# stattlab/azplugins

Measured on AMD Instinct MI355X. Metric: particle-steps/sec, PerturbedLennardJones pair force, higher is better.
Workload: dtype f64

## Files before the change

azplugins_amd/csrc/pair_tiled.hpp:

```cpp
#pragma once

#include <type_traits>

#include "pair_kernel.hpp"
#include "pair_plan.hpp"

#ifndef AZP_TILED_WAVES_PER_SIMD
#define AZP_TILED_WAVES_PER_SIMD 4
#endif

namespace azp
{
#ifdef AZP_TIMELINE
extern __device__ unsigned long long g_timeline[8 * 4 * 16384];
#endif

struct TileDyn
    {
    uint32_t n_shells;
    uint32_t stale;
    };

struct TiledKArgs
    {
    PairKArgs p;
    const uint32_t* tile_nstage;
    const uint64_t* tile_head;
    const uint32_t* stage_idx;
    const uint32_t* slice_Kend;
    uint32_t n_shells;
    const uint64_t* slice_head;
    const uint4* cnl;
    const uint8_t* perm;
    const TileDyn* dyn;
    const uint32_t* dflag;
    const unsigned long long* dbits;
    const float* disp;
    double shell_w;
    double shell_winv;
    double bound_extra;
    };

__device__ __forceinline__ float wave_max_nonneg(float v)
    {
#pragma unroll
    for (int off = 32; off > 0; off >>= 1)
        v = fmaxf(v, __shfl_xor(v, off, 64));
    return v;
    }

__device__ __forceinline__ uint32_t tile_shells_for(double b, double shell_winv)
    {
    if (!(b >= 0.0))
        return PLAN_SHELLS;
    if (b == 0.0)
        return 0u;
    if (!(shell_winv > 0.0))
        return PLAN_SHELLS;
    const double n = ceil(2.0 * b * (1.0 + 1e-9) * shell_winv);
    return n >= (double)PLAN_SHELLS ? PLAN_SHELLS : (uint32_t)n;
    }

#define AZP_TILE_STRIDE(CAP) ((CAP) + 1)

constexpr int TILE_BATCH = 4;

struct TileBatch
    {
    double x[TILE_BATCH], y[TILE_BATCH], z[TILE_BATCH];
    uint32_t off[TILE_BATCH];
    };

inline void fill_local_bound(TiledKArgs& k, const PairPlan& plan, const azp_pair_args& args)
    {
    const bool local = args.d_displacement && args.has_displacement_bound && args.displacement_bound >= 0.0;
    k.disp = local ? args.d_displacement : nullptr;
    k.dflag = (args.d_stale_flag && args.d_displacement_sq_bits) ? args.d_stale_flag : nullptr;
    k.dbits = k.dflag ? args.d_displacement_sq_bits : nullptr;
    if (k.dflag)
        k.disp = nullptr;
    k.shell_w = plan.shell_width;
    k.shell_winv = plan.shell_width > 0.0 ? 1.0 / plan.shell_width : 0.0;
    k.bound_extra = args.displacement_bound_extra > 0.0 ? args.displacement_bound_extra : 0.0;
    }

template<int CAP, int H> __device__ __forceinline__ void tile_gather(TileBatch& b, const uint4& u, const char* bx)
    {
    constexpr int NB = TILE_BATCH;
    const uint32_t w0 = H ? u.z : u.x, w1 = H ? u.w : u.y;
    b.off[0] = w0 & 0xffffu;
    b.off[1] = w0 >> 16;
    b.off[2] = w1 & 0xffffu;
    b.off[3] = w1 >> 16;
#pragma unroll
    for (int e = 0; e < NB; ++e)
        {
        b.x[e] = *reinterpret_cast<const double*>(bx + b.off[e]);
        b.y[e] = *reinterpret_cast<const double*>(bx + b.off[e] + AZP_TILE_STRIDE(CAP) * 8);
        b.z[e] = *reinterpret_cast<const double*>(bx + b.off[e] + AZP_TILE_STRIDE(CAP) * 16);
        }
    }

template<class E, int CAP, bool VIRIAL, bool SINGLE, bool XPLOR, bool WRAP>
__device__ __forceinline__ void tile_compute(const TileBatch& b, const TiledKArgs& a, const char* bt,
                                             const typename E::Coeff* __restrict__ s_coeff,
                                             const double* __restrict__ s_ronsq, const typename E::Coeff& c0, double ronsq0,
                                             double rcutsq_max, const double3& pi, int typei, double& fx, double& fy,
                                             double& fz, double& pe, double (&v)[6], uint32_t& n_core, uint32_t& n_in, double (&es)[2])
    {
    typedef typename E::Coeff Coeff;
    constexpr int NB = TILE_BATCH;
    constexpr bool SPLIT = SINGLE && !XPLOR && E::kSplitEnergy;
    double dx[NB], dy[NB], dz[NB], rsq[NB];
    bool any_in = false;
#pragma unroll
    for (int e = 0; e < NB; ++e)
        {
        dx[e] = pi.x - b.x[e]; dy[e] = pi.y - b.y[e]; dz[e] = pi.z - b.z[e];
        if (WRAP)
            min_image(a.p.box, dx[e], dy[e], dz[e]);
        rsq[e] = __builtin_fma(dz[e], dz[e], __builtin_fma(dy[e], dy[e], dx[e] * dx[e]));
        if (WRAP)
            rsq[e] = (b.off[e] == 0) ? 1.0e60 : rsq[e];
        any_in = any_in || (rsq[e] < rcutsq_max);
        }
    const bool none_in = !__any(any_in);
    if (SPLIT ? __builtin_expect(none_in, 0) : none_in)
        return;
    double fd[NB];
    if constexpr (SPLIT)
        {
        double x[NB];
        E::rcp4(rsq, x);
        bool any_core = false;
#pragma unroll
        for (int e = 0; e < NB; ++e)
            any_core = any_core || E::in_core(c0, rsq[e]);
        if (!__any(any_core))
            {
            const bool count_in = c0.tail_add != 0.0;
#pragma unroll
            for (int e = 0; e < NB; ++e)
                E::eval_split_tail(c0, rsq[e], x[e], fd[e], es[0], es[1], n_in, count_in);
            }
        else
            {
#pragma unroll
            for (int e = 0; e < NB; ++e)
                E::eval_split(c0, rsq[e], x[e], fd[e], pe, n_core, n_in);
            }
        }
#pragma unroll
    for (int e = 0; e < NB; ++e)
        {
        double force_divr, pair_eng = 0.0;
        if constexpr (SPLIT)
            force_divr = fd[e];
        else if (SINGLE)
            {
            const bool evaluated = E::eval(c0, rsq[e], force_divr, pair_eng);
            if (XPLOR && evaluated)
                apply_xplor(rsq[e], ronsq0, c0.rcutsq, force_divr, pair_eng);
            }
        else
            {
            const int typej = *reinterpret_cast<const int*>(bt + (b.off[e] >> 1));
            const uint32_t tp = (uint32_t)typei * a.p.ntypes + (uint32_t)typej;
            const Coeff cc = s_coeff[tp];
            const bool evaluated = E::eval(cc, rsq[e], force_divr, pair_eng);
            if (XPLOR && evaluated)
                apply_xplor(rsq[e], s_ronsq[tp], cc.rcutsq, force_divr, pair_eng);
            }
        fx = __builtin_fma(dx[e], force_divr, fx);
        fy = __builtin_fma(dy[e], force_divr, fy);
        fz = __builtin_fma(dz[e], force_divr, fz);
        if constexpr (!SPLIT)
            pe += pair_eng;
        if (VIRIAL)
            {
            const double fxx = force_divr * dx[e], fyy = force_divr * dy[e];
            v[0] = __builtin_fma(fxx, dx[e], v[0]);
            v[1] = __builtin_fma(fxx, dy[e], v[1]);
            v[2] = __builtin_fma(fxx, dz[e], v[2]);
            v[3] = __builtin_fma(fyy, dy[e], v[3]);
            v[4] = __builtin_fma(fyy, dz[e], v[4]);
            v[5] = __builtin_fma(force_divr * dz[e], dz[e], v[5]);
            }
        }
    }

template<class E, int TPP, int CAP, bool VIRIAL, bool SINGLE, bool XPLOR, bool WRAP>
__device__ __forceinline__ void tiled_loop(const TiledKArgs& a, const char* bx, const char* bt,
                                           const typename E::Coeff* __restrict__ s_coeff,
                                           const double* __restrict__ s_ronsq, const typename E::Coeff& c0, double ronsq0,
                                           double rcutsq_max, const char* __restrict__ slice_base, uint32_t lane_off, uint32_t Kb,
                                           double3 pi, int typei, double& fx, double& fy, double& fz, double& pe, double (&v)[6], uint32_t& n_core,
                                           uint32_t& n_in, double (&es)[2])
    {
    const uint4 zero4 = make_uint4(0, 0, 0, 0);
    auto chunk_at = [&](uint32_t kk) -> uint4
        { return *reinterpret_cast<const uint4*>(slice_base + (uint64_t)kk * 1024u + lane_off); };
    const uint32_t K = Kb >> 1;
    const uint32_t Kc = (Kb + 1u) >> 1;
    uint4 u = (Kc > 0) ? chunk_at(0) : zero4;
    uint4 un = (Kc > 1) ? chunk_at(1) : u;
    TileBatch A, B;
    tile_gather<CAP, 0>(A, u, bx);
    for (uint32_t kk = 0; kk < K; ++kk)
        {
        const uint4 un2 = chunk_at((kk + 2 < Kc) ? kk + 2 : Kc - 1);
        tile_gather<CAP, 1>(B, u, bx);
        __builtin_amdgcn_sched_barrier(0);
        tile_compute<E, CAP, VIRIAL, SINGLE, XPLOR, WRAP>(A, a, bt, s_coeff, s_ronsq, c0, ronsq0, rcutsq_max, pi, typei, fx, fy, fz, pe, v, n_core, n_in, es);
        __builtin_amdgcn_sched_barrier(0);
        tile_gather<CAP, 0>(A, un, bx);
        __builtin_amdgcn_sched_barrier(0);
        tile_compute<E, CAP, VIRIAL, SINGLE, XPLOR, WRAP>(B, a, bt, s_coeff, s_ronsq, c0, ronsq0, rcutsq_max, pi, typei, fx, fy, fz, pe, v, n_core, n_in, es);
        __builtin_amdgcn_sched_barrier(0);
        u = un;
        un = un2;
        }
    if (Kb & 1u)
        tile_compute<E, CAP, VIRIAL, SINGLE, XPLOR, WRAP>(A, a, bt, s_coeff, s_ronsq, c0, ronsq0, rcutsq_max, pi, typei, fx, fy, fz, pe, v, n_core, n_in, es);
    }

template<class E, int TPP, int CAP, bool VIRIAL, bool SINGLE, bool XPLOR>
__global__ void __launch_bounds__(256, E::kTileWaves) pair_forces_tiled_kernel(const TiledKArgs a, const typename E::Params* __restrict__ params)
    {
    typedef typename E::Coeff Coeff;
    constexpr int TB = 256 / TPP;
    constexpr int PW = 64 / TPP;
    extern __shared__ __attribute__((aligned(16))) unsigned char s_raw[];
    double* s_x = reinterpret_cast<double*>(s_raw);
    double* s_y = s_x + AZP_TILE_STRIDE(CAP);
    double* s_z = s_y + AZP_TILE_STRIDE(CAP);
    int* s_t = reinterpret_cast<int*>(s_z + AZP_TILE_STRIDE(CAP));
    Coeff* s_coeff = reinterpret_cast<Coeff*>(s_raw + (size_t)AZP_TILE_STRIDE(CAP) * 24 + (SINGLE ? 0 : (size_t)CAP * 4 + 8));
    double* s_ronsq = reinterpret_cast<double*>(s_coeff + (SINGLE ? 0 : a.p.ntypes * a.p.ntypes));

    const uint32_t tid = threadIdx.x;
    __builtin_amdgcn_s_setprio(3);
#ifdef AZP_TIMELINE
    const unsigned long long tl_t0 = __builtin_amdgcn_s_memrealtime();
    const unsigned long long tl_c0 = __builtin_amdgcn_s_memtime();
    unsigned long long tl_tb = 0, tl_tc = 0, tl_td = 0, tl_ta = 0;
#endif
    const uint32_t tile = a.p.first / TB + xcd_remap(blockIdx.x, a.p.nblocks_padded);
    const uint32_t first = tile * TB;
    if (first >= a.p.end)
        return;
    if (a.dyn && a.dyn->stale)
        return;
    if (a.dflag && *a.dflag)
        return;

    Coeff c0;
    double ronsq0 = 0.0;
    double rcutsq_max = 0.0;
    if (SINGLE)
        {
        c0 = to_uniform(prepare_coeff<E>(a.p, params, 0));
        if (XPLOR)
            ronsq0 = a.p.ronsq[0];
        rcutsq_max = c0.rcutsq;
        }
    else
        {
        const uint32_t ntp = a.p.ntypes * a.p.ntypes;
        for (uint32_t t = tid; t < ntp; t += 256)
            {
            s_coeff[t] = prepare_coeff<E>(a.p, params, t);
            s_ronsq[t] = XPLOR ? a.p.ronsq[t] : 0.0;
            }
        for (uint32_t t = 0; t < ntp; ++t)
            rcutsq_max = fmax(rcutsq_max, a.p.rcutsq[t]);
        }

#ifdef AZP_TIMELINE
    tl_ta = __builtin_amdgcn_s_memrealtime();
#endif
    const uint32_t n_stage = a.tile_nstage[tile];
    const uint32_t* __restrict__ stage = a.stage_idx + a.tile_head[tile];
    const double3 c = load_scalar3_of4(a.p.pos, first);
    if (tid == 0)
        {
        s_x[0] = PLAN_FAR; s_y[0] = PLAN_FAR; s_z[0] = PLAN_FAR;
        if (!SINGLE) s_t[0] = 0;
        }
    const uint32_t wave = (uint32_t)__builtin_amdgcn_readfirstlane((int)(tid >> 6)), lane = tid & 63;
    const uint32_t pl = lane / TPP;
    const uint32_t idx = first + ((TPP == 1 && a.perm) ? (uint32_t)a.perm[(uint64_t)tile * 256u + tid] : wave * PW + pl);
    const bool active = idx < a.p.end;
    const double4 own = load_scalar4(a.p.pos, active ? idx : first);
    const bool no_hint = !(a.p.r_list_max > 0.0);
    bool far_from_c = false;
    float dmax = a.disp ? a.disp[active ? idx : first] : 0.f;
    {
    constexpr int ROUNDS = (CAP + 255) / 256;
    uint32_t sj[ROUNDS];
#pragma unroll
    for (int r = 0; r < ROUNDS; ++r)
        {
        const uint32_t sidx = (uint32_t)r * 256u + tid;
        sj[r] = (sidx < n_stage) ? stage[sidx] : first;
        }
#ifdef AZP_TIMELINE
    __builtin_amdgcn_s_waitcnt(0);
    tl_tb = __builtin_amdgcn_s_memrealtime();
#endif
    double sxv[ROUNDS], syv[ROUNDS], szv[ROUNDS];
    int stv[ROUNDS];
    if (a.disp)
        {
#pragma unroll
        for (int r = 0; r < ROUNDS; ++r)
            dmax = fmaxf(dmax, a.disp[sj[r]]);
        }
#pragma unroll
    for (int r = 0; r < ROUNDS; ++r)
        {
        if (SINGLE)
            {
            const double3 pj = load_scalar3_of4(a.p.pos, sj[r]);
            sxv[r] = pj.x; syv[r] = pj.y; szv[r] = pj.z;
            }
        else
            {
            const double4 pj = load_scalar4(a.p.pos, sj[r]);
            sxv[r] = pj.x; syv[r] = pj.y; szv[r] = pj.z;
            stv[r] = type_from_w(pj.w);
            }
        }
#ifdef AZP_TIMELINE
    __builtin_amdgcn_s_waitcnt(0);
    tl_tc = __builtin_amdgcn_s_memrealtime();
#endif
#pragma unroll
    for (int r = 0; r < ROUNDS; ++r)
        {
        const uint32_t sidx = (uint32_t)r * 256u + tid;
        if (sidx < n_stage)
            {
            double x = sxv[r], y = syv[r], z = szv[r];
            if (!a.p.box.triclinic)
                {
                if (a.p.box.px) x = __builtin_fma(-a.p.box.Lx, rint((x - c.x) * a.p.box.Lxinv), x);
                if (a.p.box.py) y = __builtin_fma(-a.p.box.Ly, rint((y - c.y) * a.p.box.Lyinv), y);
                if (a.p.box.pz) z = __builtin_fma(-a.p.box.Lz, rint((z - c.z) * a.p.box.Lzinv), z);
                if (no_hint)
                    far_from_c = far_from_c || (a.p.box.px && fabs(x - c.x) >= 0.25 * a.p.box.Lx)
                                 || (a.p.box.py && fabs(y - c.y) >= 0.25 * a.p.box.Ly)
                                 || (a.p.box.pz && fabs(z - c.z) >= 0.25 * a.p.box.Lz);
                }
            s_x[sidx + 1] = x; s_y[sidx + 1] = y; s_z[sidx + 1] = z;
            if (!SINGLE)
                s_t[sidx + 1] = stv[r];
            }
        }
    }

    double3 pi = make_double3(0.0, 0.0, 0.0);
    int typei = 0;
    bool lane_wide = far_from_c || a.p.box.triclinic;
    if (active)
        {
        const double4 p = own;
        double x = p.x, y = p.y, z = p.z;
        if (!a.p.box.triclinic)
            {
            if (a.p.box.px) x = __builtin_fma(-a.p.box.Lx, rint((x - c.x) * a.p.box.Lxinv), x);
            if (a.p.box.py) y = __builtin_fma(-a.p.box.Ly, rint((y - c.y) * a.p.box.Lyinv), y);
            if (a.p.box.pz) z = __builtin_fma(-a.p.box.Lz, rint((z - c.z) * a.p.box.Lzinv), z);
            const double rx = no_hint ? 0.25 * a.p.box.Lx : a.p.r_list_max, ry = no_hint ? 0.25 * a.p.box.Ly : a.p.r_list_max,
                         rz = no_hint ? 0.25 * a.p.box.Lz : a.p.r_list_max;
            lane_wide = lane_wide || (a.p.box.px && fabs(x - c.x) + rx >= 0.5 * a.p.box.Lx)
                        || (a.p.box.py && fabs(y - c.y) + ry >= 0.5 * a.p.box.Ly)
                        || (a.p.box.pz && fabs(z - c.z) + rz >= 0.5 * a.p.box.Lz);
            }
        pi = make_double3(x, y, z);
        typei = type_from_w(p.w);
        }
#ifdef AZP_TIMELINE
    __builtin_amdgcn_s_waitcnt(0);
    tl_td = __builtin_amdgcn_s_memrealtime();
#endif
    __shared__ float s_dmax[4];
    if (a.disp)
        {
        dmax = wave_max_nonneg(dmax);
        if (lane == 0)
            s_dmax[wave] = dmax;
        }
    const bool wide = __syncthreads_or(lane_wide);
    __builtin_amdgcn_s_setprio(0);
#ifdef AZP_TIMELINE
    const unsigned long long tl_t1 = __builtin_amdgcn_s_memrealtime();
#endif
    uint32_t n_shells = a.dyn ? min(a.dyn->n_shells, PLAN_SHELLS) : a.n_shells;
    if (a.dbits)
        n_shells = tile_shells_for(to_uniform(sqrt(__longlong_as_double((long long)*a.dbits)) + a.bound_extra), a.shell_winv);
    if (a.disp)
        {
        const float d4 = fmaxf(fmaxf(s_dmax[0], s_dmax[1]), fmaxf(s_dmax[2], s_dmax[3]));
        n_shells = tile_shells_for(to_uniform((double)d4 + a.bound_extra), a.shell_winv);
        }

    const uint32_t slice = tile * 4 + wave;
    const uint32_t Kb = to_uniform(a.slice_Kend[(PLAN_SHELLS + 1) * slice + min(n_shells, PLAN_SHELLS)]);
    const uint64_t slice_head = to_uniform(a.slice_head[slice]);
    const char* __restrict__ slice_base = reinterpret_cast<const char*>(a.cnl + slice_head * 64ull);
    const uint32_t lane_off = lane * 16u;

    double fx = 0.0, fy = 0.0, fz = 0.0, pe = 0.0;
    double v[6] = {0.0, 0.0, 0.0, 0.0, 0.0, 0.0};
    uint32_t n_core = 0, n_in = 0;
    double es[2] = {0.0, 0.0};
    const char* bx = reinterpret_cast<const char*>(s_x);
    const char* bt = reinterpret_cast<const char*>(s_t);
    if (wide)
        tiled_loop<E, TPP, CAP, VIRIAL, SINGLE, XPLOR, true>(a, bx, bt, s_coeff, s_ronsq, c0, ronsq0, rcutsq_max, slice_base, lane_off, Kb, pi,
                                                            typei, fx, fy, fz, pe, v, n_core, n_in, es);
    else
        tiled_loop<E, TPP, CAP, VIRIAL, SINGLE, XPLOR, false>(a, bx, bt, s_coeff, s_ronsq, c0, ronsq0, rcutsq_max, slice_base, lane_off, Kb, pi,
                                                             typei, fx, fy, fz, pe, v, n_core, n_in, es);
    if constexpr (SINGLE && !XPLOR && E::kSplitEnergy)
        pe = E::finish_split(c0, pe, es[0], es[1], n_core, n_in);

#ifdef AZP_TIMELINE
    if (lane == 0 && tile < 16384)
        {
        unsigned long long* t = g_timeline + (tile * 4 + wave) * 8;
        t[4] = tl_ta; t[5] = tl_tb; t[6] = tl_tc; t[7] = tl_td;
        if (wave == 3)
            t[4] = __builtin_amdgcn_s_memtime() - tl_c0;
        t[0] = tl_t0; t[1] = tl_t1; t[2] = __builtin_amdgcn_s_memrealtime();
        t[3] = ((unsigned long long)__builtin_amdgcn_s_getreg((20 ) | (0 << 6) | (31 << 11)) << 32)
               | (unsigned)__builtin_amdgcn_s_getreg((4 ) | (0 << 6) | (31 << 11));
        }
#endif
    fx = group_sum<TPP>(fx);
    fy = group_sum<TPP>(fy);
    fz = group_sum<TPP>(fz);
    pe = group_sum<TPP>(pe);
    if (VIRIAL)
        {
#pragma unroll
        for (int cidx = 0; cidx < 6; ++cidx)
            v[cidx] = group_sum<TPP>(v[cidx]);
        }
    if (active && (lane % TPP) == 0)
        {
        store_scalar4(a.p.force, idx, fx, fy, fz, 0.5 * pe);
        if (VIRIAL)
            {
#pragma unroll
            for (int cidx = 0; cidx < 6; ++cidx)
                a.p.virial[(uint64_t)cidx * a.p.virial_pitch + idx] = 0.5 * v[cidx];
            }
        }
    }

inline TiledKArgs make_tiled_kargs(const PairPlan& plan, const azp_pair_args& args, const TileDyn* dyn, uint32_t tb)
    {
    TiledKArgs k = {};
    k.p = make_pair_kargs(args);
    k.tile_nstage = plan.d_tile_nstage;
    k.tile_head = plan.d_tile_head;
    k.stage_idx = plan.d_stage_idx;
    k.perm = plan.balanced ? plan.d_perm : nullptr;
    k.slice_Kend = plan.d_slice_Kend;
    k.n_shells = plan_shells_for(plan, args);
    fill_local_bound(k, plan, args);
    k.dyn = dyn;
    k.slice_head = plan.d_slice_head;
    k.cnl = plan.d_cnl;
    const uint32_t t0 = k.p.first / tb, t1 = (k.p.end + tb - 1) / tb;
    k.p.first = t0 * tb;
    k.p.end = (t1 * tb < args.N) ? t1 * tb : args.N;
    k.p.nblocks_padded = (t1 - t0 + 7u) & ~7u;
    return k;
    }

inline uint32_t plan_launch_cap(const PairPlan& plan, const azp_pair_args& args, uint32_t tb)
    {
    if (args.range_count == 0 || plan.h_tile_nstage.empty())
        return plan.cap;
    const uint32_t end = (args.range_first + args.range_count < args.N) ? args.range_first + args.range_count : args.N;
    const uint32_t t0 = args.range_first / tb, t1 = (end + tb - 1) / tb;
    uint32_t most = 0;
    for (uint32_t t = t0; t < t1 && t < plan.n_tiles; ++t)
        most = plan.h_tile_nstage[t] > most ? plan.h_tile_nstage[t] : most;
    return plan_cap_for(most);
    }

template<class E, int TPP, int CAP, bool VIRIAL, bool SINGLE>
int launch_tiled_instance(const PairPlan& plan, const azp_pair_args& args, const typename E::Params* d_params,
                          hipStream_t stream, const TileDyn* dyn)
    {
    const TiledKArgs k = make_tiled_kargs(plan, args, dyn, plan.tile);
    size_t lds = (size_t)AZP_TILE_STRIDE(CAP) * 24 + (SINGLE ? 0 : (size_t)CAP * 4 + 8);
    if (!SINGLE)
        lds += (sizeof(typename E::Coeff) + sizeof(double)) * (size_t)args.ntypes * args.ntypes;
    if (args.shift_mode == AZP_SHIFT_XPLOR)
        return launch_dyn_lds(pair_forces_tiled_kernel<E, TPP, CAP, VIRIAL, SINGLE, true>, k.p.nblocks_padded, 256, TPP, lds, stream, k, d_params);
    return launch_dyn_lds(pair_forces_tiled_kernel<E, TPP, CAP, VIRIAL, SINGLE, false>, k.p.nblocks_padded, 256, TPP, lds, stream, k, d_params);
    }

template<class E, int TPP, bool VIRIAL, bool SINGLE>
int launch_tiled_cap(const PairPlan& plan, const azp_pair_args& args, const typename E::Params* d_params, hipStream_t s, const TileDyn* dyn)
    {
    const uint32_t cap = plan_launch_cap(plan, args, plan.tile);
    switch (cap)
        {
    case 1024: return launch_tiled_instance<E, TPP, 1024, VIRIAL, SINGLE>(plan, args, d_params, s, dyn);
    case 1536: return launch_tiled_instance<E, TPP, 1536, VIRIAL, SINGLE>(plan, args, d_params, s, dyn);
    case 1664: return launch_tiled_instance<E, TPP, 1664, VIRIAL, SINGLE>(plan, args, d_params, s, dyn);
    case 2048: return launch_tiled_instance<E, TPP, 2048, VIRIAL, SINGLE>(plan, args, d_params, s, dyn);
    case 2560: return launch_tiled_instance<E, TPP, 2560, VIRIAL, SINGLE>(plan, args, d_params, s, dyn);
    default: return AZP_ERROR_INVALID_ARGUMENT;
        }
    }

template<class E>
int launch_tiled_tpp(const PairPlan& plan, const azp_pair_args& args, const typename E::Params* d_params, hipStream_t s, const TileDyn* dyn)
    {
    const bool single = (args.ntypes == 1);
    auto go = [&](auto t)
        {
        constexpr int TPP = decltype(t)::value;
        if (args.compute_virial)
            return single ? launch_tiled_cap<E, TPP, true, true>(plan, args, d_params, s, dyn)
                          : launch_tiled_cap<E, TPP, true, false>(plan, args, d_params, s, dyn);
        return single ? launch_tiled_cap<E, TPP, false, true>(plan, args, d_params, s, dyn)
                      : launch_tiled_cap<E, TPP, false, false>(plan, args, d_params, s, dyn);
        };
    switch (plan.tpp)
        {
    case 1: return go(std::integral_constant<int, 1>());
    case 2: return go(std::integral_constant<int, 2>());
    case 4: return go(std::integral_constant<int, 4>());
    default: return AZP_ERROR_INVALID_ARGUMENT;
        }
    }

}
```

Before: 9.013 billion.

## Add specialized single-type tiled path with core/tail phase split and fast staging

Adds a dedicated kernel path for TPP=1 single-type split-energy potentials that loads tile metadata through scalar (constant address space) loads, uses a fast periodic staging path with 32-bit offsets, and splits the neighbor chunk loop into a core phase and a tail phase. Chunks beyond a per-slice Kphase index are known to lie outside the WCA core given the displacement bound, so the tail phase skips the per-batch core test and wave vote. This cuts branch and vote overhead in the inner loop and setup latency, at the cost of more code, extra plan data (slice_Kphase) and a correctness dependence on the host-computed core reach bound.

```diff
diff --git a/azplugins_amd/csrc/pair_tiled.hpp b/azplugins_amd/csrc/pair_tiled.hpp
--- a/azplugins_amd/csrc/pair_tiled.hpp
+++ b/azplugins_amd/csrc/pair_tiled.hpp
@@ -39,6 +39,9 @@
     double shell_w;
     double shell_winv;
     double bound_extra;
+    const uint32_t* slice_Kphase;
+    double core_reach_sq;
+    uint32_t fast_stage;
     };
 
 __device__ __forceinline__ float wave_max_nonneg(float v)
@@ -59,6 +62,26 @@
         return PLAN_SHELLS;
     const double n = ceil(2.0 * b * (1.0 + 1e-9) * shell_winv);
     return n >= (double)PLAN_SHELLS ? PLAN_SHELLS : (uint32_t)n;
+    }
+
+template<class T> __device__ __forceinline__ T load_uniform(const T* p)
+    {
+    return *(const __attribute__((address_space(4))) T*)p;
+    }
+
+__device__ __forceinline__ double4 load_scalar4_o32(const double* base, uint32_t idx)
+    {
+    const char* p = reinterpret_cast<const char*>(base) + (idx << 5);
+    const double2 a = *reinterpret_cast<const double2*>(p);
+    const double2 b = *reinterpret_cast<const double2*>(p + 16);
+    return make_double4(a.x, a.y, b.x, b.y);
+    }
+__device__ __forceinline__ double3 load_scalar3_of4_o32(const double* base, uint32_t idx)
+    {
+    const char* p = reinterpret_cast<const char*>(base) + (idx << 5);
+    const double2 a = *reinterpret_cast<const double2*>(p);
+    const double z = *reinterpret_cast<const double*>(p + 16);
+    return make_double3(a.x, a.y, z);
     }
 
 #define AZP_TILE_STRIDE(CAP) ((CAP) + 1)
@@ -101,7 +124,7 @@
         }
     }
 
-template<class E, int CAP, bool VIRIAL, bool SINGLE, bool XPLOR, bool WRAP>
+template<class E, int CAP, bool VIRIAL, bool SINGLE, bool XPLOR, bool WRAP, bool TAIL = false>
 __device__ __forceinline__ void tile_compute(const TileBatch& b, const TiledKArgs& a, const char* bt,
                                              const typename E::Coeff* __restrict__ s_coeff,
                                              const double* __restrict__ s_ronsq, const typename E::Coeff& c0, double ronsq0,
@@ -133,15 +156,24 @@
         double x[NB];
         E::rcp4(rsq, x);
         bool any_core = false;
-#pragma unroll
-        for (int e = 0; e < NB; ++e)
-            any_core = any_core || E::in_core(c0, rsq[e]);
-        if (!__any(any_core))
+        if constexpr (!TAIL)
+            {
+#pragma unroll
+            for (int e = 0; e < NB; ++e)
+                any_core = any_core || E::in_core(c0, rsq[e]);
+            }
+        if (TAIL || !__any(any_core))
             {
             const bool count_in = c0.tail_add != 0.0;
 #pragma unroll
             for (int e = 0; e < NB; ++e)
-                E::eval_split_tail(c0, rsq[e], x[e], fd[e], es[0], es[1], n_in, count_in);
+                E::eval_split_tail(c0, rsq[e], x[e], fd[e], es[0], es[1], n_in, TAIL ? false : count_in);
+            if (TAIL && __builtin_expect(count_in, 0))
+                {
+#pragma unroll
+                for (int e = 0; e < NB; ++e)
+                    n_in += (rsq[e] < c0.rcutsq) ? 1u : 0u;
+                }
             }
         else
             {
@@ -224,240 +256,524 @@
         tile_compute<E, CAP, VIRIAL, SINGLE, XPLOR, WRAP>(A, a, bt, s_coeff, s_ronsq, c0, ronsq0, rcutsq_max, pi, typei, fx, fy, fz, pe, v, n_core, n_in, es);
     }
 
+template<class E, int TPP, int CAP, bool VIRIAL>
+__device__ __forceinline__ void tiled_loop_phases(const TiledKArgs& a, const char* bx, const typename E::Coeff& c0, double rcutsq_max,
+                                                  const char* __restrict__ slice_base, uint32_t lane_off, uint32_t Kb, uint32_t Kcore,
+                                                  double3 pi, int typei, double& fx, double& fy, double& fz, double& pe, double (&v)[6],
+                                                  uint32_t& n_core, uint32_t& n_in, double (&es)[2])
+    {
+    const uint4 zero4 = make_uint4(0, 0, 0, 0);
+    auto chunk_at = [&](uint32_t kk) -> uint4
+        { return *reinterpret_cast<const uint4*>(slice_base + (uint64_t)kk * 1024u + lane_off); };
+    const uint32_t K = Kb >> 1;
+    const uint32_t Kc = (Kb + 1u) >> 1;
+    uint4 u = (Kc > 0) ? chunk_at(0) : zero4;
+    uint4 un = (Kc > 1) ? chunk_at(1) : u;
+    TileBatch A, B;
+    tile_gather<CAP, 0>(A, u, bx);
+    auto iteration = [&](auto tail_tag, const uint32_t kk)
+        {
+        constexpr bool TAIL = decltype(tail_tag)::value;
+        const uint4 un2 = chunk_at((kk + 2 < Kc) ? kk + 2 : Kc - 1);
+        tile_gather<CAP, 1>(B, u, bx);
+        __builtin_amdgcn_sched_barrier(0);
+        tile_compute<E, CAP, VIRIAL, true, false, false, TAIL>(A, a, nullptr, nullptr, nullptr, c0, 0.0, rcutsq_max, pi, typei, fx, fy, fz, pe, v, n_core, n_in, es);
+        __builtin_amdgcn_sched_barrier(0);
+        tile_gather<CAP, 0>(A, un, bx);
+        __builtin_amdgcn_sched_barrier(0);
+        tile_compute<E, CAP, VIRIAL, true, false, false, TAIL>(B, a, nullptr, nullptr, nullptr, c0, 0.0, rcutsq_max, pi, typei, fx, fy, fz, pe, v, n_core, n_in, es);
+        __builtin_amdgcn_sched_barrier(0);
+        u = un;
+        un = un2;
+        };
+    const uint32_t K1 = (Kcore < K) ? Kcore : K;
+    for (uint32_t kk = 0; kk < K1; ++kk)
+        iteration(std::false_type(), kk);
+    for (uint32_t kk = K1; kk < K; ++kk)
+        iteration(std::true_type(), kk);
+    if (Kb & 1u)
+        tile_compute<E, CAP, VIRIAL, true, false, false>(A, a, nullptr, nullptr, nullptr, c0, 0.0, rcutsq_max, pi, typei, fx, fy, fz, pe, v, n_core, n_in, es);
+    }
 template<class E, int TPP, int CAP, bool VIRIAL, bool SINGLE, bool XPLOR>
 __global__ void __launch_bounds__(256, E::kTileWaves) pair_forces_tiled_kernel(const TiledKArgs a, const typename E::Params* __restrict__ params)
     {
-    typedef typename E::Coeff Coeff;
-    constexpr int TB = 256 / TPP;
-    constexpr int PW = 64 / TPP;
-    extern __shared__ __attribute__((aligned(16))) unsigned char s_raw[];
-    double* s_x = reinterpret_cast<double*>(s_raw);
-    double* s_y = s_x + AZP_TILE_STRIDE(CAP);
-    double* s_z = s_y + AZP_TILE_STRIDE(CAP);
-    int* s_t = reinterpret_cast<int*>(s_z + AZP_TILE_STRIDE(CAP));
-    Coeff* s_coeff = reinterpret_cast<Coeff*>(s_raw + (size_t)AZP_TILE_STRIDE(CAP) * 24 + (SINGLE ? 0 : (size_t)CAP * 4 + 8));
-    double* s_ronsq = reinterpret_cast<double*>(s_coeff + (SINGLE ? 0 : a.p.ntypes * a.p.ntypes));
-
-    const uint32_t tid = threadIdx.x;
-    __builtin_amdgcn_s_setprio(3);
-#ifdef AZP_TIMELINE
-    const unsigned long long tl_t0 = __builtin_amdgcn_s_memrealtime();
-    const unsigned long long tl_c0 = __builtin_amdgcn_s_memtime();
-    unsigned long long tl_tb = 0, tl_tc = 0, tl_td = 0, tl_ta = 0;
-#endif
-    const uint32_t tile = a.p.first / TB + xcd_remap(blockIdx.x, a.p.nblocks_padded);
-    const uint32_t first = tile * TB;
-    if (first >= a.p.end)
-        return;
-    if (a.dyn && a.dyn->stale)
-        return;
-    if (a.dflag && *a.dflag)
-        return;
-
-    Coeff c0;
-    double ronsq0 = 0.0;
-    double rcutsq_max = 0.0;
-    if (SINGLE)
-        {
-        c0 = to_uniform(prepare_coeff<E>(a.p, params, 0));
-        if (XPLOR)
-            ronsq0 = a.p.ronsq[0];
-        rcutsq_max = c0.rcutsq;
+    if constexpr (TPP == 1 && SINGLE && !XPLOR && E::kSplitEnergy)
+        {
+        typedef typename E::Coeff Coeff;
+        constexpr int TB = 256;
+        extern __shared__ __attribute__((aligned(16))) unsigned char s_raw[];
+        double* s_x = reinterpret_cast<double*>(s_raw);
+        double* s_y = s_x + AZP_TILE_STRIDE(CAP);
+        double* s_z = s_y + AZP_TILE_STRIDE(CAP);
+
+        const uint32_t tid = threadIdx.x;
+        __builtin_amdgcn_s_setprio(3);
+#ifdef AZP_TIMELINE
+        const unsigned long long tl_t0 = __builtin_amdgcn_s_memrealtime();
+        const unsigned long long tl_c0 = __builtin_amdgcn_s_memtime();
+        unsigned long long tl_tb = 0, tl_tc = 0, tl_td = 0, tl_ta = 0;
+#endif
+        const uint32_t tile = a.p.first / TB + xcd_remap(blockIdx.x, a.p.nblocks_padded);
+        const uint32_t first = tile * TB;
+        if (first >= a.p.end)
+            return;
+        const uint32_t wave = (uint32_t)__builtin_amdgcn_readfirstlane((int)(tid >> 6)), lane = tid & 63;
+        const uint32_t slice = tile * 4 + wave;
+
+        const uint32_t n_stage = load_uniform(a.tile_nstage + tile);
+        const uint64_t stage_head = load_uniform(a.tile_head + tile);
+        asm volatile("" ::"s"(n_stage), "s"(stage_head));
+        const uint32_t* __restrict__ stage = a.stage_idx + stage_head;
+        const uint32_t* spare = a.tile_nstage + tile;
+        const uint32_t w_stale = load_uniform(a.dyn ? &a.dyn->stale : spare);
+        const uint32_t w_shells = load_uniform(a.dyn ? &a.dyn->n_shells : spare);
+        const uint32_t w_flag = load_uniform(a.dflag ? a.dflag : spare);
+        const unsigned long long w_bits = load_uniform(a.dbits ? a.dbits : reinterpret_cast<const unsigned long long*>(a.tile_head + tile));
+        const double3 c = make_double3(load_uniform(a.p.pos + 4ull * first), load_uniform(a.p.pos + 4ull * first + 1),
+                                       load_uniform(a.p.pos + 4ull * first + 2));
+        const uint64_t slice_head = load_uniform(a.slice_head + slice);
+        const uint8_t member = *(a.perm ? a.perm + ((uint64_t)tile * 256u + tid) : reinterpret_cast<const uint8_t*>(spare));
+        constexpr int ROUNDS = (CAP + 255) / 256;
+        uint32_t sj[ROUNDS];
+#pragma unroll
+        for (int r = 0; r < ROUNDS; ++r)
+            {
+            const uint32_t sidx = (uint32_t)r * 256u + tid;
+            sj[r] = (sidx < n_stage) ? stage[sidx] : first;
+            }
+        __builtin_amdgcn_sched_barrier(0);
+        const uint32_t idx = first + (a.perm ? (uint32_t)member : wave * 64u + lane);
+        const bool active = idx < a.p.end;
+        if (((a.dyn != nullptr) & (w_stale != 0u)) | ((a.dflag != nullptr) & (w_flag != 0u)))
+            return;
+#ifdef AZP_TIMELINE
+        __builtin_amdgcn_s_waitcnt(0);
+        tl_tb = __builtin_amdgcn_s_memrealtime();
+#endif
+        uint32_t n_shells = a.dyn ? min(w_shells, PLAN_SHELLS) : a.n_shells;
+        if (a.dbits)
+            n_shells = tile_shells_for(to_uniform(sqrt(__longlong_as_double((long long)w_bits)) + a.bound_extra), a.shell_winv);
+        uint32_t Kb = load_uniform(a.slice_Kend + ((PLAN_SHELLS + 1) * slice + min(n_shells, PLAN_SHELLS)));
+        uint32_t Kcore = load_uniform(a.core_reach_sq > 0.0 ? a.slice_Kphase + slice : spare);
+
+        const Coeff c0 = to_uniform(E::prepare(params[0], load_uniform(a.p.rcutsq), a.p.shift_mode == AZP_SHIFT_SHIFT));
+        const double rcutsq_max = c0.rcutsq;
+        if (!(a.core_reach_sq > 0.0 && c0.wca_rsq <= a.core_reach_sq))
+            Kcore = 0xffffffffu;
+        asm volatile("" ::"s"(c.x), "s"(c.y), "s"(c.z), "s"(slice_head), "s"(Kb), "s"(Kcore), "s"(a.fast_stage), "s"(a.p.pos));
+        __builtin_amdgcn_sched_barrier(0);
+#ifdef AZP_TIMELINE
+        tl_ta = __builtin_amdgcn_s_memrealtime();
+#endif
+        if (tid == 0)
+            {
+            s_x[0] = PLAN_FAR; s_y[0] = PLAN_FAR; s_z[0] = PLAN_FAR;
+            }
+
+        double3 pi = make_double3(0.0, 0.0, 0.0);
+        bool lane_wide = false;
+        float dmax = 0.f;
+        const uint32_t me = active ? idx : first;
+        if (a.disp)
+            {
+            dmax = a.disp[me];
+#pragma unroll
+            for (int r = 0; r < ROUNDS; ++r)
+                dmax = fmaxf(dmax, a.disp[sj[r]]);
+            }
+        double sxv[ROUNDS], syv[ROUNDS], szv[ROUNDS];
+        if (a.fast_stage)
+            {
+            const double3 own = load_scalar3_of4_o32(a.p.pos, me);
+#pragma unroll
+            for (int r = 0; r < ROUNDS; ++r)
+                {
+                const double3 pj = load_scalar3_of4_o32(a.p.pos, sj[r]);
+                sxv[r] = pj.x; syv[r] = pj.y; szv[r] = pj.z;
+                }
+#ifdef AZP_TIMELINE
+            __builtin_amdgcn_s_waitcnt(0);
+            tl_tc = __builtin_amdgcn_s_memrealtime();
+#endif
+#pragma unroll
+            for (int r = 0; r < ROUNDS; ++r)
+                {
+                const uint32_t sidx = (uint32_t)r * 256u + tid;
+                if (sidx < n_stage)
+                    {
+                    s_x[sidx + 1] = __builtin_fma(-a.p.box.Lx, rint((sxv[r] - c.x) * a.p.box.Lxinv), sxv[r]);
+                    s_y[sidx + 1] = __builtin_fma(-a.p.box.Ly, rint((syv[r] - c.y) * a.p.box.Lyinv), syv[r]);
+                    s_z[sidx + 1] = __builtin_fma(-a.p.box.Lz, rint((szv[r] - c.z) * a.p.box.Lzinv), szv[r]);
+                    }
+                }
+            if (active)
+                {
+                const double x = __builtin_fma(-a.p.box.Lx, rint((own.x - c.x) * a.p.box.Lxinv), own.x);
+                const double y = __builtin_fma(-a.p.box.Ly, rint((own.y - c.y) * a.p.box.Lyinv), own.y);
+                const double z = __builtin_fma(-a.p.box.Lz, rint((own.z - c.z) * a.p.box.Lzinv), own.z);
+                lane_wide = (fabs(x - c.x) + a.p.r_list_max >= 0.5 * a.p.box.Lx) || (fabs(y - c.y) + a.p.r_list_max >= 0.5 * a.p.box.Ly)
+                            || (fabs(z - c.z) + a.p.r_list_max >= 0.5 * a.p.box.Lz);
+                pi = make_double3(x, y, z);
+                }
+            }
+        else
+            {
+            const double3 own = load_scalar3_of4(a.p.pos, me);
+            const bool no_hint = !(a.p.r_list_max > 0.0);
+            bool far_from_c = false;
+#pragma unroll
+            for (int r = 0; r < ROUNDS; ++r)
+                {
+                const double3 pj = load_scalar3_of4(a.p.pos, sj[r]);
+                sxv[r] = pj.x; syv[r] = pj.y; szv[r] = pj.z;
+                }
+#ifdef AZP_TIMELINE
+            __builtin_amdgcn_s_waitcnt(0);
+            tl_tc = __builtin_amdgcn_s_memrealtime();
+#endif
+#pragma unroll
+            for (int r = 0; r < ROUNDS; ++r)
+                {
+                const uint32_t sidx = (uint32_t)r * 256u + tid;
+                if (sidx < n_stage)
+                    {
+                    double x = sxv[r], y = syv[r], z = szv[r];
+                    if (!a.p.box.triclinic)
+                        {
+                        if (a.p.box.px) x = __builtin_fma(-a.p.box.Lx, rint((x - c.x) * a.p.box.Lxinv), x);
+                        if (a.p.box.py) y = __builtin_fma(-a.p.box.Ly, rint((y - c.y) * a.p.box.Lyinv), y);
+                        if (a.p.box.pz) z = __builtin_fma(-a.p.box.Lz, rint((z - c.z) * a.p.box.Lzinv), z);
+                        if (no_hint)
+                            far_from_c = far_from_c || (a.p.box.px && fabs(x - c.x) >= 0.25 * a.p.box.Lx)
+                                         || (a.p.box.py && fabs(y - c.y) >= 0.25 * a.p.box.Ly)
+                                         || (a.p.box.pz && fabs(z - c.z) >= 0.25 * a.p.box.Lz);
+                        }
+                    s_x[sidx + 1] = x; s_y[sidx + 1] = y; s_z[sidx + 1] = z;
+                    }
+                }
+            lane_wide = far_from_c || a.p.box.triclinic;
+            if (active)
+                {
+                double x = own.x, y = own.y, z = own.z;
+                if (!a.p.box.triclinic)
+                    {
+                    if (a.p.box.px) x = __builtin_fma(-a.p.box.Lx, rint((x - c.x) * a.p.box.Lxinv), x);
+                    if (a.p.box.py) y = __builtin_fma(-a.p.box.Ly, rint((y - c.y) * a.p.box.Lyinv), y);
+                    if (a.p.box.pz) z = __builtin_fma(-a.p.box.Lz, rint((z - c.z) * a.p.box.Lzinv), z);
+                    const double rx = no_hint ? 0.25 * a.p.box.Lx : a.p.r_list_max, ry = no_hint ? 0.25 * a.p.box.Ly : a.p.r_list_max,
+                                 rz = no_hint ? 0.25 * a.p.box.Lz : a.p.r_list_max;
+                    lane_wide = lane_wide || (a.p.box.px && fabs(x - c.x) + rx >= 0.5 * a.p.box.Lx)
+                                || (a.p.box.py && fabs(y - c.y) + ry >= 0.5 * a.p.box.Ly)
+                                || (a.p.box.pz && fabs(z - c.z) + rz >= 0.5 * a.p.box.Lz);
+                    }
+                pi = make_double3(x, y, z);
+                }
+            }
+#ifdef AZP_TIMELINE
+        __builtin_amdgcn_s_waitcnt(0);
+        tl_td = __builtin_amdgcn_s_memrealtime();
+#endif
+        __shared__ float s_dmax[4];
+        if (a.disp)
+            {
+            dmax = wave_max_nonneg(dmax);
+            if (lane == 0)
+                s_dmax[wave] = dmax;
+            }
+        const bool wide = __syncthreads_or(lane_wide);
+        __builtin_amdgcn_s_setprio(0);
+#ifdef AZP_TIMELINE
+        const unsigned long long tl_t1 = __builtin_amdgcn_s_memrealtime();
+#endif
+        if (a.disp)
+            {
+            const float d4 = fmaxf(fmaxf(s_dmax[0], s_dmax[1]), fmaxf(s_dmax[2], s_dmax[3]));
+            const uint32_t tile_shells = tile_shells_for(to_uniform((double)d4 + a.bound_extra), a.shell_winv);
+            Kb = to_uniform(a.slice_Kend[(PLAN_SHELLS + 1) * slice + min(tile_shells, PLAN_SHELLS)]);
+            }
+        const char* __restrict__ slice_base = reinterpret_cast<const char*>(a.cnl + slice_head * 64ull);
+        const uint32_t lane_off = lane * 16u;
+
+        double fx = 0.0, fy = 0.0, fz = 0.0, pe = 0.0;
+        double v[6] = {0.0, 0.0, 0.0, 0.0, 0.0, 0.0};
+        uint32_t n_core = 0, n_in = 0;
+        double es[2] = {0.0, 0.0};
+        const char* bx = reinterpret_cast<const char*>(s_x);
+        if (wide)
+            tiled_loop<E, 1, CAP, VIRIAL, true, false, true>(a, bx, nullptr, nullptr, nullptr, c0, 0.0, rcutsq_max, slice_base, lane_off, Kb, pi, 0,
+                                                             fx, fy, fz, pe, v, n_core, n_in, es);
+        else
+            tiled_loop_phases<E, 1, CAP, VIRIAL>(a, bx, c0, rcutsq_max, slice_base, lane_off, Kb, Kcore, pi, 0, fx, fy, fz, pe, v, n_core,
+                                                 n_in, es);
+        pe = E::finish_split(c0, pe, es[0], es[1], n_core, n_in);
+
+#ifdef AZP_TIMELINE
+        if (lane == 0 && tile < 16384)
+            {
+            unsigned long long* t = g_timeline + (tile * 4 + wave) * 8;
+            t[4] = tl_ta; t[5] = tl_tb; t[6] = tl_tc; t[7] = tl_td;
+            if (wave == 3)
+                t[4] = __builtin_amdgcn_s_memtime() - tl_c0;
+            t[0] = tl_t0; t[1] = tl_t1; t[2] = __builtin_amdgcn_s_memrealtime();
+            t[3] = ((unsigned long long)__builtin_amdgcn_s_getreg((20 ) | (0 << 6) | (31 << 11)) << 32)
+                   | (unsigned)__builtin_amdgcn_s_getreg((4 ) | (0 << 6) | (31 << 11));
+            }
+#endif
+        if (active)
+            {
+            store_scalar4(a.p.force, idx, fx, fy, fz, 0.5 * pe);
+            if (VIRIAL)
+                {
+#pragma unroll
+                for (int cidx = 0; cidx < 6; ++cidx)
+                    a.p.virial[(uint64_t)cidx * a.p.virial_pitch + idx] = 0.5 * v[cidx];
+                }
+            }
         }
     else
         {
-        const uint32_t ntp = a.p.ntypes * a.p.ntypes;
-        for (uint32_t t = tid; t < ntp; t += 256)
-            {
-            s_coeff[t] = prepare_coeff<E>(a.p, params, t);
-            s_ronsq[t] = XPLOR ? a.p.ronsq[t] : 0.0;
-            }
-        for (uint32_t t = 0; t < ntp; ++t)
-            rcutsq_max = fmax(rcutsq_max, a.p.rcutsq[t]);
-        }
-
-#ifdef AZP_TIMELINE
-    tl_ta = __builtin_amdgcn_s_memrealtime();
-#endif
-    const uint32_t n_stage = a.tile_nstage[tile];
-    const uint32_t* __restrict__ stage = a.stage_idx + a.tile_head[tile];
-    const double3 c = load_scalar3_of4(a.p.pos, first);
-    if (tid == 0)
-        {
-        s_x[0] = PLAN_FAR; s_y[0] = PLAN_FAR; s_z[0] = PLAN_FAR;
-        if (!SINGLE) s_t[0] = 0;
-        }
-    const uint32_t wave = (uint32_t)__builtin_amdgcn_readfirstlane((int)(tid >> 6)), lane = tid & 63;
-    const uint32_t pl = lane / TPP;
-    const uint32_t idx = first + ((TPP == 1 && a.perm) ? (uint32_t)a.perm[(uint64_t)tile * 256u + tid] : wave * PW + pl);
-    const bool active = idx < a.p.end;
-    const double4 own = load_scalar4(a.p.pos, active ? idx : first);
-    const bool no_hint = !(a.p.r_list_max > 0.0);
-    bool far_from_c = false;
-    float dmax = a.disp ? a.disp[active ? idx : first] : 0.f;
-    {
-    constexpr int ROUNDS = (CAP + 255) / 256;
-    uint32_t sj[ROUNDS];
-#pragma unroll
-    for (int r = 0; r < ROUNDS; ++r)
-        {
-        const uint32_t sidx = (uint32_t)r * 256u + tid;
-        sj[r] = (sidx < n_stage) ? stage[sidx] : first;
-        }
-#ifdef AZP_TIMELINE
-    __builtin_amdgcn_s_waitcnt(0);
-    tl_tb = __builtin_amdgcn_s_memrealtime();
-#endif
-    double sxv[ROUNDS], syv[ROUNDS], szv[ROUNDS];
-    int stv[ROUNDS];
-    if (a.disp)
-        {
+        typedef typename E::Coeff Coeff;
+        constexpr int TB = 256 / TPP;
+        constexpr int PW = 64 / TPP;
+        extern __shared__ __attribute__((aligned(16))) unsigned char s_raw[];
+        double* s_x = reinterpret_cast<double*>(s_raw);
+        double* s_y = s_x + AZP_TILE_STRIDE(CAP);
+        double* s_z = s_y + AZP_TILE_STRIDE(CAP);
+        int* s_t = reinterpret_cast<int*>(s_z + AZP_TILE_STRIDE(CAP));
+        Coeff* s_coeff = reinterpret_cast<Coeff*>(s_raw + (size_t)AZP_TILE_STRIDE(CAP) * 24 + (SINGLE ? 0 : (size_t)CAP * 4 + 8));
+        double* s_ronsq = reinterpret_cast<double*>(s_coeff + (SINGLE ? 0 : a.p.ntypes * a.p.ntypes));
+
+        const uint32_t tid = threadIdx.x;
+        __builtin_amdgcn_s_setprio(3);
+#ifdef AZP_TIMELINE
+        const unsigned long long tl_t0 = __builtin_amdgcn_s_memrealtime();
+        const unsigned long long tl_c0 = __builtin_amdgcn_s_memtime();
+        unsigned long long tl_tb = 0, tl_tc = 0, tl_td = 0, tl_ta = 0;
+#endif
+        const uint32_t tile = a.p.first / TB + xcd_remap(blockIdx.x, a.p.nblocks_padded);
+        const uint32_t first = tile * TB;
+        if (first >= a.p.end)
+            return;
+        if (a.dyn && a.dyn->stale)
+            return;
+        if (a.dflag && *a.dflag)
+            return;
+
+        Coeff c0;
+        double ronsq0 = 0.0;
+        double rcutsq_max = 0.0;
+        if (SINGLE)
+            {
+            c0 = to_uniform(prepare_coeff<E>(a.p, params, 0));
+            if (XPLOR)
+                ronsq0 = a.p.ronsq[0];
+            rcutsq_max = c0.rcutsq;
+            }
+        else
+            {
+            const uint32_t ntp = a.p.ntypes * a.p.ntypes;
+            for (uint32_t t = tid; t < ntp; t += 256)
+                {
+                s_coeff[t] = prepare_coeff<E>(a.p, params, t);
+                s_ronsq[t] = XPLOR ? a.p.ronsq[t] : 0.0;
+                }
+            for (uint32_t t = 0; t < ntp; ++t)
+                rcutsq_max = fmax(rcutsq_max, a.p.rcutsq[t]);
+            }
+
+#ifdef AZP_TIMELINE
+        tl_ta = __builtin_amdgcn_s_memrealtime();
+#endif
+        const uint32_t n_stage = a.tile_nstage[tile];
+        const uint32_t* __restrict__ stage = a.stage_idx + a.tile_head[tile];
+        const double3 c = load_scalar3_of4(a.p.pos, first);
+        if (tid == 0)
+            {
+            s_x[0] = PLAN_FAR; s_y[0] = PLAN_FAR; s_z[0] = PLAN_FAR;
+            if (!SINGLE) s_t[0] = 0;
+            }
+        const uint32_t wave = (uint32_t)__builtin_amdgcn_readfirstlane((int)(tid >> 6)), lane = tid & 63;
+        const uint32_t pl = lane / TPP;
+        const uint32_t idx = first + ((TPP == 1 && a.perm) ? (uint32_t)a.perm[(uint64_t)tile * 256u + tid] : wave * PW + pl);
+        const bool active = idx < a.p.end;
+        const double4 own = load_scalar4(a.p.pos, active ? idx : first);
+        const bool no_hint = !(a.p.r_list_max > 0.0);
+        bool far_from_c = false;
+        float dmax = a.disp ? a.disp[active ? idx : first] : 0.f;
+        {
+        constexpr int ROUNDS = (CAP + 255) / 256;
+        uint32_t sj[ROUNDS];
 #pragma unroll
         for (int r = 0; r < ROUNDS; ++r)
-            dmax = fmaxf(dmax, a.disp[sj[r]]);
-        }
-#pragma unroll
-    for (int r = 0; r < ROUNDS; ++r)
-        {
-        if (SINGLE)
-            {
-            const double3 pj = load_scalar3_of4(a.p.pos, sj[r]);
-            sxv[r] = pj.x; syv[r] = pj.y; szv[r] = pj.z;
-            }
-        else
-            {
-            const double4 pj = load_scalar4(a.p.pos, sj[r]);
-            sxv[r] = pj.x; syv[r] = pj.y; szv[r] = pj.z;
-            stv[r] = type_from_w(pj.w);
-            }
-        }
-#ifdef AZP_TIMELINE
-    __builtin_amdgcn_s_waitcnt(0);
-    tl_tc = __builtin_amdgcn_s_memrealtime();
-#endif
-#pragma unroll
-    for (int r = 0; r < ROUNDS; ++r)
-        {
-        const uint32_t sidx = (uint32_t)r * 256u + tid;
-        if (sidx < n_stage)
-            {
-            double x = sxv[r], y = syv[r], z = szv[r];
+            {
+            const uint32_t sidx = (uint32_t)r * 256u + tid;
+            sj[r] = (sidx < n_stage) ? stage[sidx] : first;
+            }
+#ifdef AZP_TIMELINE
+        __builtin_amdgcn_s_waitcnt(0);
+        tl_tb = __builtin_amdgcn_s_memrealtime();
+#endif
+        double sxv[ROUNDS], syv[ROUNDS], szv[ROUNDS];
+        int stv[ROUNDS];
+        if (a.disp)
+            {
+#pragma unroll
+            for (int r = 0; r < ROUNDS; ++r)
+                dmax = fmaxf(dmax, a.disp[sj[r]]);
+            }
+#pragma unroll
+        for (int r = 0; r < ROUNDS; ++r)
+            {
+            if (SINGLE)
+                {
+                const double3 pj = load_scalar3_of4(a.p.pos, sj[r]);
+                sxv[r] = pj.x; syv[r] = pj.y; szv[r] = pj.z;
+                }
+            else
+                {
+                const double4 pj = load_scalar4(a.p.pos, sj[r]);
+                sxv[r] = pj.x; syv[r] = pj.y; szv[r] = pj.z;
+                stv[r] = type_from_w(pj.w);
+                }
+            }
+#ifdef AZP_TIMELINE
+        __builtin_amdgcn_s_waitcnt(0);
+        tl_tc = __builtin_amdgcn_s_memrealtime();
+#endif
+#pragma unroll
+        for (int r = 0; r < ROUNDS; ++r)
+            {
+            const uint32_t sidx = (uint32_t)r * 256u + tid;
+            if (sidx < n_stage)
+                {
+                double x = sxv[r], y = syv[r], z = szv[r];
+                if (!a.p.box.triclinic)
+                    {
+                    if (a.p.box.px) x = __builtin_fma(-a.p.box.Lx, rint((x - c.x) * a.p.box.Lxinv), x);
+                    if (a.p.box.py) y = __builtin_fma(-a.p.box.Ly, rint((y - c.y) * a.p.box.Lyinv), y);
+                    if (a.p.box.pz) z = __builtin_fma(-a.p.box.Lz, rint((z - c.z) * a.p.box.Lzinv), z);
+                    if (no_hint)
+                        far_from_c = far_from_c || (a.p.box.px && fabs(x - c.x) >= 0.25 * a.p.box.Lx)
+                                     || (a.p.box.py && fabs(y - c.y) >= 0.25 * a.p.box.Ly)
+                                     || (a.p.box.pz && fabs(z - c.z) >= 0.25 * a.p.box.Lz);
+                    }
+                s_x[sidx + 1] = x; s_y[sidx + 1] = y; s_z[sidx + 1] = z;
+                if (!SINGLE)
+                    s_t[sidx + 1] = stv[r];
+                }
+            }
+        }
+
+        double3 pi = make_double3(0.0, 0.0, 0.0);
+        int typei = 0;
+        bool lane_wide = far_from_c || a.p.box.triclinic;
+        if (active)
+            {
+            const double4 p = own;
+            double x = p.x, y = p.y, z = p.z;
             if (!a.p.box.triclinic)
                 {
                 if (a.p.box.px) x = __builtin_fma(-a.p.box.Lx, rint((x - c.x) * a.p.box.Lxinv), x);
                 if (a.p.box.py) y = __builtin_fma(-a.p.box.Ly, rint((y - c.y) * a.p.box.Lyinv), y);
                 if (a.p.box.pz) z = __builtin_fma(-a.p.box.Lz, rint((z - c.z) * a.p.box.Lzinv), z);
-                if (no_hint)
-                    far_from_c = far_from_c || (a.p.box.px && fabs(x - c.x) >= 0.25 * a.p.box.Lx)
-                                 || (a.p.box.py && fabs(y - c.y) >= 0.25 * a.p.box.Ly)
-                                 || (a.p.box.pz && fabs(z - c.z) >= 0.25 * a.p.box.Lz);
-                }
-            s_x[sidx + 1] = x; s_y[sidx + 1] = y; s_z[sidx + 1] = z;
-            if (!SINGLE)
-                s_t[sidx + 1] = stv[r];
-            }
-        }
-    }
-
-    double3 pi = make_double3(0.0, 0.0, 0.0);
-    int typei = 0;
-    bool lane_wide = far_from_c || a.p.box.triclinic;
-    if (active)
-        {
-        const double4 p = own;
-        double x = p.x, y = p.y, z = p.z;
-        if (!a.p.box.triclinic)
-            {
-            if (a.p.box.px) x = __builtin_fma(-a.p.box.Lx, rint((x - c.x) * a.p.box.Lxinv), x);
-            if (a.p.box.py) y = __builtin_fma(-a.p.box.Ly, rint((y - c.y) * a.p.box.Lyinv), y);
-            if (a.p.box.pz) z = __builtin_fma(-a.p.box.Lz, rint((z - c.z) * a.p.box.Lzinv), z);
-            const double rx = no_hint ? 0.25 * a.p.box.Lx : a.p.r_list_max, ry = no_hint ? 0.25 * a.p.box.Ly : a.p.r_list_max,
-                         rz = no_hint ? 0.25 * a.p.box.Lz : a.p.r_list_max;
-            lane_wide = lane_wide || (a.p.box.px && fabs(x - c.x) + rx >= 0.5 * a.p.box.Lx)
-                        || (a.p.box.py && fabs(y - c.y) + ry >= 0.5 * a.p.box.Ly)
-                        || (a.p.box.pz && fabs(z - c.z) + rz >= 0.5 * a.p.box.Lz);
-            }
-        pi = make_double3(x, y, z);
-        typei = type_from_w(p.w);
-        }
-#ifdef AZP_TIMELINE
-    __builtin_amdgcn_s_waitcnt(0);
-    tl_td = __builtin_amdgcn_s_memrealtime();
-#endif
-    __shared__ float s_dmax[4];
-    if (a.disp)
-        {
-        dmax = wave_max_nonneg(dmax);
-        if (lane == 0)
-            s_dmax[wave] = dmax;
-        }
-    const bool wide = __syncthreads_or(lane_wide);
-    __builtin_amdgcn_s_setprio(0);
-#ifdef AZP_TIMELINE
-    const unsigned long long tl_t1 = __builtin_amdgcn_s_memrealtime();
-#endif
-    uint32_t n_shells = a.dyn ? min(a.dyn->n_shells, PLAN_SHELLS) : a.n_shells;
-    if (a.dbits)
-        n_shells = tile_shells_for(to_uniform(sqrt(__longlong_as_double((long long)*a.dbits)) + a.bound_extra), a.shell_winv);
-    if (a.disp)
-        {
-        const float d4 = fmaxf(fmaxf(s_dmax[0], s_dmax[1]), fmaxf(s_dmax[2], s_dmax[3]));
-        n_shells = tile_shells_for(to_uniform((double)d4 + a.bound_extra), a.shell_winv);
-        }
-
-    const uint32_t slice = tile * 4 + wave;
-    const uint32_t Kb = to_uniform(a.slice_Kend[(PLAN_SHELLS + 1) * slice + min(n_shells, PLAN_SHELLS)]);
-    const uint64_t slice_head = to_uniform(a.slice_head[slice]);
-    const char* __restrict__ slice_base = reinterpret_cast<const char*>(a.cnl + slice_head * 64ull);
-    const uint32_t lane_off = lane * 16u;
-
-    double fx = 0.0, fy = 0.0, fz = 0.0, pe = 0.0;
-    double v[6] = {0.0, 0.0, 0.0, 0.0, 0.0, 0.0};
-    uint32_t n_core = 0, n_in = 0;
-    double es[2] = {0.0, 0.0};
-    const char* bx = reinterpret_cast<const char*>(s_x);
-    const char* bt = reinterpret_cast<const char*>(s_t);
-    if (wide)
-        tiled_loop<E, TPP, CAP, VIRIAL, SINGLE, XPLOR, true>(a, bx, bt, s_coeff, s_ronsq, c0, ronsq0, rcutsq_max, slice_base, lane_off, Kb, pi,
-                                                            typei, fx, fy, fz, pe, v, n_core, n_in, es);
-    else
-        tiled_loop<E, TPP, CAP, VIRIAL, SINGLE, XPLOR, false>(a, bx, bt, s_coeff, s_ronsq, c0, ronsq0, rcutsq_max, slice_base, lane_off, Kb, pi,
-                                                             typei, fx, fy, fz, pe, v, n_core, n_in, es);
-    if constexpr (SINGLE && !XPLOR && E::kSplitEnergy)
-        pe = E::finish_split(c0, pe, es[0], es[1], n_core, n_in);
-
-#ifdef AZP_TIMELINE
-    if (lane == 0 && tile < 16384)
-        {
-        unsigned long long* t = g_timeline + (tile * 4 + wave) * 8;
-        t[4] = tl_ta; t[5] = tl_tb; t[6] = tl_tc; t[7] = tl_td;
-        if (wave == 3)
-            t[4] = __builtin_amdgcn_s_memtime() - tl_c0;
-        t[0] = tl_t0; t[1] = tl_t1; t[2] = __builtin_amdgcn_s_memrealtime();
-        t[3] = ((unsigned long long)__builtin_amdgcn_s_getreg((20 ) | (0 << 6) | (31 << 11)) << 32)
-               | (unsigned)__builtin_amdgcn_s_getreg((4 ) | (0 << 6) | (31 << 11));
-        }
-#endif
-    fx = group_sum<TPP>(fx);
-    fy = group_sum<TPP>(fy);
-    fz = group_sum<TPP>(fz);
-    pe = group_sum<TPP>(pe);
-    if (VIRIAL)
-        {
-#pragma unroll
-        for (int cidx = 0; cidx < 6; ++cidx)
-            v[cidx] = group_sum<TPP>(v[cidx]);
-        }
-    if (active && (lane % TPP) == 0)
-        {
-        store_scalar4(a.p.force, idx, fx, fy, fz, 0.5 * pe);
+                const double rx = no_hint ? 0.25 * a.p.box.Lx : a.p.r_list_max, ry = no_hint ? 0.25 * a.p.box.Ly : a.p.r_list_max,
+                             rz = no_hint ? 0.25 * a.p.box.Lz : a.p.r_list_max;
+                lane_wide = lane_wide || (a.p.box.px && fabs(x - c.x) + rx >= 0.5 * a.p.box.Lx)
+                            || (a.p.box.py && fabs(y - c.y) + ry >= 0.5 * a.p.box.Ly)
+                            || (a.p.box.pz && fabs(z - c.z) + rz >= 0.5 * a.p.box.Lz);
+                }
+            pi = make_double3(x, y, z);
+            typei = type_from_w(p.w);
+            }
+#ifdef AZP_TIMELINE
+        __builtin_amdgcn_s_waitcnt(0);
+        tl_td = __builtin_amdgcn_s_memrealtime();
+#endif
+        __shared__ float s_dmax[4];
+        if (a.disp)
+            {
+            dmax = wave_max_nonneg(dmax);
+            if (lane == 0)
+                s_dmax[wave] = dmax;
+            }
+        const bool wide = __syncthreads_or(lane_wide);
+        __builtin_amdgcn_s_setprio(0);
+#ifdef AZP_TIMELINE
+        const unsigned long long tl_t1 = __builtin_amdgcn_s_memrealtime();
+#endif
+        uint32_t n_shells = a.dyn ? min(a.dyn->n_shells, PLAN_SHELLS) : a.n_shells;
+        if (a.dbits)
+            n_shells = tile_shells_for(to_uniform(sqrt(__longlong_as_double((long long)*a.dbits)) + a.bound_extra), a.shell_winv);
+        if (a.disp)
+            {
+            const float d4 = fmaxf(fmaxf(s_dmax[0], s_dmax[1]), fmaxf(s_dmax[2], s_dmax[3]));
+            n_shells = tile_shells_for(to_uniform((double)d4 + a.bound_extra), a.shell_winv);
+            }
+
+        const uint32_t slice = tile * 4 + wave;
+        const uint32_t Kb = to_uniform(a.slice_Kend[(PLAN_SHELLS + 1) * slice + min(n_shells, PLAN_SHELLS)]);
+        const uint64_t slice_head = to_uniform(a.slice_head[slice]);
+        const char* __restrict__ slice_base = reinterpret_cast<const char*>(a.cnl + slice_head * 64ull);
+        const uint32_t lane_off = lane * 16u;
+
+        double fx = 0.0, fy = 0.0, fz = 0.0, pe = 0.0;
+        double v[6] = {0.0, 0.0, 0.0, 0.0, 0.0, 0.0};
+        uint32_t n_core = 0, n_in = 0;
+        double es[2] = {0.0, 0.0};
+        const char* bx = reinterpret_cast<const char*>(s_x);
+        const char* bt = reinterpret_cast<const char*>(s_t);
+        if (wide)
+            tiled_loop<E, TPP, CAP, VIRIAL, SINGLE, XPLOR, true>(a, bx, bt, s_coeff, s_ronsq, c0, ronsq0, rcutsq_max, slice_base, lane_off, Kb, pi,
+                                                                typei, fx, fy, fz, pe, v, n_core, n_in, es);
+        else
+            tiled_loop<E, TPP, CAP, VIRIAL, SINGLE, XPLOR, false>(a, bx, bt, s_coeff, s_ronsq, c0, ronsq0, rcutsq_max, slice_base, lane_off, Kb, pi,
+                                                                 typei, fx, fy, fz, pe, v, n_core, n_in, es);
+        if constexpr (SINGLE && !XPLOR && E::kSplitEnergy)
+            pe = E::finish_split(c0, pe, es[0], es[1], n_core, n_in);
+
+#ifdef AZP_TIMELINE
+        if (lane == 0 && tile < 16384)
+            {
+            unsigned long long* t = g_timeline + (tile * 4 + wave) * 8;
+            t[4] = tl_ta; t[5] = tl_tb; t[6] = tl_tc; t[7] = tl_td;
+            if (wave == 3)
+                t[4] = __builtin_amdgcn_s_memtime() - tl_c0;
+            t[0] = tl_t0; t[1] = tl_t1; t[2] = __builtin_amdgcn_s_memrealtime();
+            t[3] = ((unsigned long long)__builtin_amdgcn_s_getreg((20 ) | (0 << 6) | (31 << 11)) << 32)
+                   | (unsigned)__builtin_amdgcn_s_getreg((4 ) | (0 << 6) | (31 << 11));
+            }
+#endif
+        fx = group_sum<TPP>(fx);
+        fy = group_sum<TPP>(fy);
+        fz = group_sum<TPP>(fz);
+        pe = group_sum<TPP>(pe);
         if (VIRIAL)
             {
 #pragma unroll
             for (int cidx = 0; cidx < 6; ++cidx)
-                a.p.virial[(uint64_t)cidx * a.p.virial_pitch + idx] = 0.5 * v[cidx];
-            }
-        }
+                v[cidx] = group_sum<TPP>(v[cidx]);
+            }
+        if (active && (lane % TPP) == 0)
+            {
+            store_scalar4(a.p.force, idx, fx, fy, fz, 0.5 * pe);
+            if (VIRIAL)
+                {
+#pragma unroll
+                for (int cidx = 0; cidx < 6; ++cidx)
+                    a.p.virial[(uint64_t)cidx * a.p.virial_pitch + idx] = 0.5 * v[cidx];
+                }
+            }
+        }
+    }
+
+inline double plan_core_reach_sq(const PairPlan& plan, const azp_pair_args& args, const TiledKArgs& k)
+    {
+    if (!(plan.core_r > 0.f) || !plan.d_slice_Kphase || k.dyn || k.dflag || k.disp)
+        return 0.0;
+    if (!args.has_displacement_bound || !(args.displacement_bound >= 0.0))
+        return 0.0;
+    const double reach = (double)plan.core_r - 2.0 * (args.displacement_bound + k.bound_extra) * (1.0 + 1e-9);
+    return reach > 0.0 ? reach * reach * (1.0 - 1e-12) : 0.0;
     }
 
 inline TiledKArgs make_tiled_kargs(const PairPlan& plan, const azp_pair_args& args, const TileDyn* dyn, uint32_t tb)
@@ -474,6 +790,9 @@
     k.dyn = dyn;
     k.slice_head = plan.d_slice_head;
     k.cnl = plan.d_cnl;
+    k.slice_Kphase = plan.d_slice_Kphase;
+    k.core_reach_sq = plan_core_reach_sq(plan, args, k);
+    k.fast_stage = (!k.p.box.triclinic && k.p.box.px && k.p.box.py && k.p.box.pz && k.p.r_list_max > 0.0 && args.n_max < (1u << 27)) ? 1u : 0u;
     const uint32_t t0 = k.p.first / tb, t1 = (k.p.end + tb - 1) / tb;
     k.p.first = t0 * tb;
     k.p.end = (t1 * tb < args.N) ? t1 * tb : args.N;
```

Result: faster. 9.399 billion, median of 6 (+4.3%).
